# nikhilTkur/Multigrid_dolfinx

Measured on AMD Instinct MI355X. Metric: V-cycles/sec + achieved HBM GB/s, 3D Poisson P1 1024³ DoF, 1/2/4/8 MI355X, higher is better.
Workload: dtype f64

## Files before the change

multigrid_dolfinx_amd/csrc/mg_capi.hip:

```cpp
#include "../../include/mg_hip.h"
#include "mg_csr_check.h"
#include "mg_kernels.hip.h"
#include "mg_direct.hip.h"
#include "mg_jacobi2.hip.h"
#include "mg_jacobik3d.hip.h"
#include "mg_jacobiblk.hip.h"
#include "mg_lattice.hip.h"
#include "mg_diffusion_mf.hip.h"
#include "mg_diffusion_adj.hip.h"
#include "mg_diffusion_kappa.hip.h"

#include <dlfcn.h>
#include <rccl/rccl.h>

#include <algorithm>
#include <array>
#include <cmath>
#include <cstdio>
#include <cstdlib>
#include <cstring>
#include <string>
#include <type_traits>
#include <vector>

// ... 216 lines not shown
    double *pcg_r = nullptr, *pcg_z = nullptr, *pcg_q = nullptr, *pcg_part_a = nullptr, *pcg_part_b = nullptr;
    DVector pcg_p;
    int pcg_parts = 0, pcg_parts_a = 0;
    int pcg_predict = 0;
    double* fcg_work = nullptr;
    double* fcg_spmv = nullptr;
    int64_t fcg_work_n = 0, fcg_spmv_n = 0;
    int use_graph = 1;
    int comm_priority = 1;
    int lattice_march = 1;
    int64_t lattice_march_min_rows = 1 << 22;
    int lattice_gs2 = 0;
    int diffusion_faces = MG_FACES_ALL;
    int dkappa_gather = 0;
    int lattice_tile = 0;
    int lattice_segments = 0;
    int slab_pair_form = 0;
    int graph_comm = 0;
    uint64_t epoch = 1;
    std::vector<CycleGraph> graphs;
    bool capturing = false;
    int use_direct = 1;
    int require_diagonal = 1;
    int fuse_restrict = 1;
    int fuse_block = 1;
    int64_t fuse_block_min_rows = (int64_t)1 << 15, fuse_block_max_rows = (int64_t)1 << 23;
    int fuse_block_k = 0, fuse_block_ez = 11;
    int direct_block_rows = 2048;
    int fuse_2d_lines = 0;
    int gen_odd_rows = 0;
    int cls_escape = 1;
    int storage_auto = 1;
    int storage_qbits = 0;
    int use_classes = 1;
    int fuse_sweeps = 1;
    int64_t fuse_min_rows = (int64_t)1 << 24;
    int fuse_segments = 0;
    int fuse_nontemporal = 0;
    int fuse_classes = 1;
    int fuse_plain_shape = 0;
    int fuse_plain = 2;
    int class_sweeps = 1;
    int fuse_k = 5;
    int fuse_k_shape = -1;
    int fuse_k_segments = 0;
    int timing_force_form = -1;
    int64_t fuse_k_slab_min_rows = (int64_t)1 << 20;
    int fuse_k_slab_min_sweeps = 4;
    int64_t fuse_k_min_rows = (int64_t)1 << 24;
    int64_t fuse_k_small_rows = (int64_t)1 << 22;
    int64_t fuse_k5_min_rows = (int64_t)1 << 26;
    int64_t fuse_k4_min_rows = 0;
    int fuse_k_nt_store = 0;
    int fuse_k_tail = 1;
    int fuse_k_small_tiles = 0;
    int fuse_k_pf = 1;
    int fuse_k_dpp = 1;
    std::vector<const void*> large_lds_kernels;
    int fuse_shape = 1;
    int fuse_wi = 0;
    int fuse_even = 0;
    int march_sweeps = 1;
    int64_t march_min_rows = (int64_t)1 << 22;
    int march_shape = 0;
    int64_t fuse_small_2d_rows = 2048;
    int fuse_small = 1;
    int fuse_2d = 1;
    int fuse_2d_k = 5;
    int fuse_xcd_chunk = 32;
    int cls_blocks_per_cu = 4;
    DirectSolver direct;
    int* ptab_count = nullptr;
    int p1_prolong = 0;
    int* rtab_count = nullptr;
    int* rtab_off = nullptr;
    double* rtab_w = nullptr;
    int rtab_m = 0;
    int* ptab_off = nullptr;
    double* ptab_w = nullptr;
    Level mass;
    int mass_level = -1;
    DVector mass_out, diff, uexact;
    int uexact_level = -1;
    int64_t uploads = 0, downloads = 0, graph_replays = 0;
    struct SmootherCount { int64_t launches = 0, sweeps = 0, tail = 0; };
    std::vector<std::array<SmootherCount, MG_PATH_COUNT>> smoother_counts;
    int jk3_tail = 0;
    double* stage = nullptr;
    int64_t stage_elems = 0;
    int64_t bytes = 0;
    Comm comm;
    hipDeviceProp_t prop{};
};

namespace {

constexpr int kMaxParts = 1024;

template <class T>
int dev_alloc(mg_context* c, T** p, size_t count) {
    *p = nullptr;
    if (count == 0) count = 1;
    HIP_TRY(hipMalloc(reinterpret_cast<void**>(p), count * sizeof(T)));
    c->bytes += (int64_t)(count * sizeof(T));
    return 0;
}
// ... 692 lines not shown
    HIP_TRY(hipStreamSynchronize(c->stream));
    if (cm.ar(cm.user, cm.h_stage, count) != 0) return fail("allreduce callback failed");
    HIP_TRY(hipMemcpyAsync(dev, cm.h_stage, (size_t)count * 8, hipMemcpyHostToDevice, c->stream));
    HIP_TRY(hipStreamSynchronize(c->stream));
    return 0;
}

int allgather_planes(mg_context* c, const std::vector<int>& splits, int64_t plane, double* full) {
    Comm& cm = c->comm;
    if (!cm.active()) return 0;
    if (cm.nccl) {
        NCCL_TRY(g_rccl.GroupStart());
        for (int r = 0; r < cm.world; ++r) {
            double* seg = full + (int64_t)splits[r] * plane;
            const size_t cnt = (size_t)(splits[r + 1] - splits[r]) * (size_t)plane;
            NCCL_TRY(g_rccl.Broadcast(seg, seg, cnt, ncclDouble, r, cm.nccl, c->stream));
        }
        NCCL_TRY(g_rccl.GroupEnd());
        return 0;
    }
    if (!cm.ag) return fail("no transport configured");
    const int64_t total = (int64_t)splits[cm.world] * plane;
    const int64_t mine = (int64_t)(splits[cm.rank + 1] - splits[cm.rank]) * plane;
    MG_TRY(ensure_host_stage(c, (size_t)(total + mine)));
    double* h_send = cm.h_stage + total;
    HIP_TRY(hipMemcpyAsync(h_send, full + (int64_t)splits[cm.rank] * plane, (size_t)mine * 8, hipMemcpyDeviceToHost,
                           c->stream));
    HIP_TRY(hipStreamSynchronize(c->stream));
    std::vector<int64_t> counts(cm.world);
    for (int r = 0; r < cm.world; ++r) counts[r] = (int64_t)(splits[r + 1] - splits[r]) * plane;
    if (cm.ag(cm.user, h_send, mine, cm.h_stage, counts.data()) != 0) return fail("allgatherv callback failed");
    HIP_TRY(hipMemcpyAsync(full, cm.h_stage, (size_t)total * 8, hipMemcpyHostToDevice, c->stream));
    HIP_TRY(hipStreamSynchronize(c->stream));
    return 0;
}

DVector* pick(Level& L, int which) {
    switch (which) {
        case MG_VEC_V: return &L.v;
        case MG_VEC_F: return &L.f;
        case MG_VEC_R: return &L.v2;
        case MG_VEC_ERR: return &L.err;
        default: return nullptr;
    }
}

int64_t min_slab_rows(const Level& L) {
    if (L.replicated || L.splits.size() < 2) return L.nloc;
    int nk = INT32_MAX;
    for (size_t r = 0; r + 1 < L.splits.size(); ++r) nk = std::min(nk, L.splits[r + 1] - L.splits[r]);
    return (int64_t)nk * L.g.plane;
}

bool fused_sweeps_ok(const mg_context* c, const Level& L, bool ignore_size = false) {
    if (!c->fuse_sweeps || !L.sdia || L.wu != 4 || L.flat) return false;
    if (L.g.nx < 32 || L.g.ny < 32 || min_slab_rows(L) < 8 * L.g.plane) return false;
    if (L.up[1] != 1 || L.up[2] != L.g.nx || (int64_t)L.up[3] != L.g.plane) return false;
    return ignore_size || min_slab_rows(L) >= c->fuse_min_rows;
}

int launch_lat_gs2(mg_context* c, const Level& L, int c1, int c2, const double* xold_rows, double* xnew_rows) {
    Gs2Args a{};
    a.xold = xold_rows; a.xnew = xnew_rows; a.f = L.f.rows;
    a.cls = L.scls; a.s_pack = L.s_pack; a.s_val = L.s_val; a.s_cnt = L.s_cnt;
    a.W = L.W; a.WP = (L.W + 3) / 4 * 4 + 4; a.ntop = L.lm_ntop;
    for (int t = 0; t < LM_K; ++t) a.top[t] = L.lm_top[t];
    a.nloc = L.nloc; a.P = L.g.plane; a.nx = L.g.nx; a.ny = L.g.ny; a.nz = L.g.nk;
    a.c1 = c1; a.c2 = c2; a.omega = c->omega;
    a.ntx = (L.g.nx + G2_TI - 1) / G2_TI; a.nty = (L.g.ny + G2_TJ - 1) / G2_TJ;
    const int64_t ntile = (int64_t)a.ntx * a.nty;
    const int64_t resident = 2 * (int64_t)std::max(1, c->prop.multiProcessorCount);
    int nseg = c->lattice_segments;
    if (nseg <= 0 && 2 * ntile >= resident) nseg = (int)std::max<int64_t>(1, (13 * resident / 2 + ntile - 1) / ntile);
    if (nseg <= 0) nseg = best_segments(ntile, resident, L.g.nk, L.g.nk / 16, 12.0);
    nseg = std::max(1, std::min(nseg, std::max(1, L.g.nk / 16)));
    a.seglen = (L.g.nk + nseg - 1) / nseg;
    nseg = (L.g.nk + a.seglen - 1) / a.seglen;
    const int64_t items = ntile * nseg;
    a.xcd_chunk = 16;
    unsigned grid = 0;
    MG_TRY(tile_grid(items, a.xcd_chunk, &grid));
    a.nitems = (unsigned)items;
    const size_t lds = g2_lds_bytes(L.W);
    if (lds > (size_t)80 * 1024) return fail("lattice march: class tables too wide");
    MG_TRY(allow_large_lds(c, reinterpret_cast<const void*>(lat_gs2), (size_t)80 * 1024));
    hipLaunchKernelGGL(lat_gs2, dim3(grid), dim3(G2_THREADS), lds, c->stream, a);
    HIP_TRY(hipGetLastError());
    return 0;
}

int allow_large_lds(mg_context* c, const void* kernel, size_t bytes) {
    if (std::find(c->large_lds_kernels.begin(), c->large_lds_kernels.end(), kernel) != c->large_lds_kernels.end()) return 0;
    HIP_TRY(hipFuncSetAttribute(kernel, hipFuncAttributeMaxDynamicSharedMemorySize, (int)bytes));
    c->large_lds_kernels.push_back(kernel);
    return 0;
}

constexpr int kJ2Lines = 16;

struct J2Plan { int ntx, nty, nseg, zb, seglen, wi; };

int jacobi2_lines(const mg_context* c, const Level& L) {
    const int sh = c->fuse_shape;
    if (!(cls_full(L) && c->fuse_classes)) return (c->fuse_plain == 2 && c->fuse_plain_shape == 0) ? 12 : kJ2Lines;
    return (sh == 1 || sh == 3) ? 24 : kJ2Lines;
}

J2Plan jacobi2_plan(const mg_context* c, const Level& L, bool slab, int64_t boundary_rows) {
    J2Plan p{};
// ... 167 lines not shown
    HIP_TRY(hipStreamSynchronize(c->stream));
    std::vector<int> map(512, 0);
    int ncls = L.ncls;
    bool grown = false;
    for (int side = 0; side < 2 && ok; ++side) {
        if (!(side == 0 ? lo : hi)) continue;
        const double* t = theirs.data() + (size_t)side * nt;
        const int n_theirs = (int)t[0];
        if (n_theirs <= 0 || n_theirs > 256) { ok = 0; break; }
        for (int j = 0; j < n_theirs && ok; ++j) {
            const double* row = t + 8 + (size_t)j * CLS_W;
            int found = -1;
            for (int i = 0; i < ncls && found < 0; ++i)
                if (std::memcmp(mine.data() + 8 + (size_t)i * CLS_W, row, 7 * sizeof(double)) == 0) found = i;
            if (found < 0) {
                if (ncls >= 256) { ok = 0; break; }
                std::memcpy(mine.data() + 8 + (size_t)ncls * CLS_W, row, 7 * sizeof(double));
                mine[8 + (size_t)ncls * CLS_W + 7] = 0.0;
                found = ncls++;
                grown = true;
            }
            map[(size_t)side * 256 + j] = found;
        }
    }
    double flag = ok ? 0.0 : 1.0;
    HIP_TRY(hipMemcpyAsync(c->scalars + 7, &flag, sizeof(double), hipMemcpyHostToDevice, c->stream));
    MG_TRY(allreduce_sum(c, c->scalars + 7, 1));
    HIP_TRY(hipMemcpyAsync(&flag, c->scalars + 7, sizeof(double), hipMemcpyDeviceToHost, c->stream));
    HIP_TRY(hipStreamSynchronize(c->stream));
    if (flag != 0.0) return 0;
    if (grown) {
        HIP_TRY(hipMemcpyAsync(L.ctab, mine.data() + 8, 256 * CLS_W * sizeof(double), hipMemcpyHostToDevice, c->stream));
        L.ncls = ncls;
    }
    HIP_TRY(hipMemcpyAsync(dmap.p, map.data(), 512 * sizeof(int), hipMemcpyHostToDevice, c->stream));
    const int* dm = reinterpret_cast<const int*>(dmap.p);
    if (lo) hipLaunchKernelGGL(doubles_to_classes, dim3(nb), dim3(256), 0, c->stream, recv.p, dm, L.cls + L.cls_lead - (int64_t)n, (int64_t)n);
    if (hi) hipLaunchKernelGGL(doubles_to_classes, dim3(nb), dim3(256), 0, c->stream, recv.p + n, dm + 256, L.cls + L.cls_lead + L.nloc, (int64_t)n);
    HIP_TRY(hipGetLastError());
    HIP_TRY(hipStreamSynchronize(c->stream));
    L.cls_halo = 1;
    return 0;
}

bool sweepsk_ok(const mg_context* c, const Level& L, bool ignore_size = false) {
    if (c->fuse_k < 3 || !L.cls || !c->fuse_classes) return false;
    if (L.cls_escape) {
        if (L.esc_kmax < 3) return false;
        ignore_size = true;
    }
    const bool slab = is_slab(c, L);
    if (slab && (L.hd < 2 || L.cls_halo < 0 || c->halo_planes != 1)) return false;
    if (!ignore_size && (slab ? min_slab_rows(L) < c->fuse_k_slab_min_rows : L.nloc < c->fuse_k_min_rows)) return false;
    return fused_sweeps_ok(c, L, true) && L.g.nk >= 8;
}

int sweepsk_max(const mg_context* c, const Level& L) {
    const int k = std::min(std::min(c->fuse_k, 5), L.nloc < c->fuse_k4_min_rows ? 3 : L.nloc < c->fuse_k_small_rows ? 5 : L.nloc < c->fuse_k5_min_rows ? 4 : 5);
    return L.cls_escape ? std::min(k, L.esc_kmax) : k;
}

template <int K>
int escape_window_k(mg_context* c, const Level& L, const unsigned char* cls, int64_t clead, unsigned* most) {
    constexpr int WI = 64 - 2 * K, HY = 16 * 2 - 2 * K + 2;
    JK3WindowArgs a{};
    a.cls = cls; a.clead = clead; a.P = L.g.plane; a.nx = L.g.nx; a.ny = L.g.ny; a.nz = L.g.nk;
    a.ntx = (a.nx + WI - 1) / WI; a.nty = (a.ny + HY - 1) / HY;
    a.most = reinterpret_cast<unsigned*>(c->partials);
    HIP_TRY(hipMemsetAsync(a.most, 0, sizeof(unsigned), c->stream));
    hipLaunchKernelGGL((jk3_escape_window<K, 16, 2, 1>), dim3((unsigned)(a.ntx * a.nty)), dim3(256), 0, c->stream, a);
    HIP_TRY(hipGetLastError());
    HIP_TRY(hipMemcpyAsync(most, a.most, sizeof(unsigned), hipMemcpyDeviceToHost, c->stream));
    HIP_TRY(hipStreamSynchronize(c->stream));
    if (std::getenv("MG_DEBUG_STORAGE"))
        std::fprintf(stderr, "[mg] escape rows: at most %u in %d planes of a tile (%d sweeps per pass, pool of %d)\n", *most, K + 2, K, jk3_pool(K));
    return 0;
}

int escape_kmax(mg_context* c, const Level& L, const unsigned char* cls, int64_t clead, int* kmax) {
    *kmax = 0;
    if (L.wu != 4 || L.g.nk < 8 || L.g.nx < 32 || L.g.ny < 32) return 0;
    unsigned most = 0;
    MG_TRY(escape_window_k<5>(c, L, cls, clead, &most));
    if (most <= (unsigned)jk3_pool(5)) { *kmax = 5; return 0; }
    MG_TRY(escape_window_k<4>(c, L, cls, clead, &most));
    if (most <= (unsigned)jk3_pool(4)) { *kmax = 4; return 0; }
    MG_TRY(escape_window_k<3>(c, L, cls, clead, &most));
    if (most <= (unsigned)jk3_pool(3)) *kmax = 3;
    return 0;
}

struct JK3Range { int za0, za1, zb0, zb1; };

int jk3_shape(const mg_context* c, int K) {
    return c->fuse_k_shape >= 0 ? c->fuse_k_shape : (K >= 5 ? 8 : 7);
}

template <int K, int NW, int LPW, int M, bool DPP, int PF = 1, int WPE = (NW == 12 ? 3 : 2), int TR = 256, bool ESC = false, bool B1 = false>
int launch_jacobikc_t(mg_context* c, JK3Args a, bool finest, const JK3Range& zr, int seglen) {
    constexpr int EX = 64 * M, EY = NW * LPW, WI = EX - 2 * K, HY = EY - 2 * K + 2;
    a.ntx = (a.nx + WI - 1) / WI;
    a.nty = (a.ny + HY - 1) / HY;
    const int64_t ntile = (int64_t)a.ntx * a.nty;
    constexpr size_t lds = B1 ? jk3b_lds_bytes<K, NW, LPW, M, TR>() : jk3_lds_bytes<K, NW, LPW, M, TR, ESC>();
    static_assert(lds <= 160 * 1024, "one CU's LDS");
    a.za0 = zr.za0; a.za1 = zr.za1; a.zb0 = zr.zb0; a.zb1 = zr.zb1;
    const int planes = std::max(0, zr.za1 - zr.za0) + std::max(0, zr.zb1 - zr.zb0);
// ... 2329 lines not shown
    } else if (k == "lattice_march") {
        c->lattice_march = value != 0;
    } else if (k == "lattice_march_min_rows") {
        c->lattice_march_min_rows = value;
    } else if (k == "dkappa_gather") {
        c->dkappa_gather = value != 0;
    } else if (k == "lattice_gs2") {
        c->lattice_gs2 = value != 0;
    } else if (k == "lattice_tile") {
        if (value < 0 || value > 2) return fail("lattice_tile must be 0, 1 or 2");
        c->lattice_tile = (int)value;
    } else if (k == "lattice_segments") {
        if (value < 0 || value > 4096) return fail("lattice_segments must be in 0..4096");
        c->lattice_segments = (int)value;
    } else if (k == "fuse_xcd_chunk") {
        if (value < 1 || value > 512) return fail("fuse_xcd_chunk must be in 1..512");
        c->fuse_xcd_chunk = (int)value;
    } else if (k == "cls_blocks_per_cu") {
        if (value < 1 || value > 64) return fail("cls_blocks_per_cu must be in 1..64");
        c->cls_blocks_per_cu = (int)value;
    } else if (k == "fuse_wi") {
        c->fuse_wi = (int)value;
    } else if (k == "fuse_even") {
        c->fuse_even = value != 0;
    } else if (k == "class_sweeps") {
        c->class_sweeps = value != 0;
    } else if (k == "fuse_plain_shape") {
        if (value < 0 || value > 2) return fail("fuse_plain_shape must be 0..2");
        c->fuse_plain_shape = (int)value;
    } else if (k == "fuse_plain") {
        if (value != 1 && value != 2) return fail("fuse_plain must be 1 or 2");
        c->fuse_plain = (int)value;
    } else if (k == "fuse_k") {
        if (value < 0 || value > 5) return fail("fuse_k must be in 0..5 (below 3: pairs of sweeps only)");
        c->fuse_k = (int)value;
    } else if (k == "fuse_k_shape") {
        if (value < -1 || value > 8) return fail("fuse_k_shape must be 0..8, or -1 (by sweeps per pass)");
        c->fuse_k_shape = (int)value;
    } else if (k == "fuse_k_slab_min_rows") {
        c->fuse_k_slab_min_rows = value;
    } else if (k == "fuse_k_slab_min_sweeps") {
        if (value < 2) return fail("fuse_k_slab_min_sweeps must be at least 2");
        c->fuse_k_slab_min_sweeps = (int)value;
    } else if (k == "fuse_k_min_rows") {
        c->fuse_k_min_rows = value;
    } else if (k == "fuse_k_small_rows") {
        c->fuse_k_small_rows = value;
    } else if (k == "fuse_k5_min_rows") {
        c->fuse_k5_min_rows = value;
    } else if (k == "fuse_k4_min_rows") {
        c->fuse_k4_min_rows = value;
    } else if (k == "fuse_k_nt_store") {
        c->fuse_k_nt_store = value != 0;
    } else if (k == "fuse_k_tail") {
        if (value < 0) return fail("fuse_k_tail must be >= 0");
        c->fuse_k_tail = (int)value;
    } else if (k == "fuse_k_small_tiles") {
        c->fuse_k_small_tiles = value != 0;
    } else if (k == "fuse_k_pf") {
        if (value != 1 && value != 2) return fail("fuse_k_pf must be 1 or 2");
        c->fuse_k_pf = (int)value;
    } else if (k == "fuse_k_dpp") {
        c->fuse_k_dpp = value != 0;
    } else if (k == "fuse_k_segments") {
        if (value < 0) return fail("fuse_k_segments must be >= 0");
        c->fuse_k_segments = (int)value;
    } else if (k == "fuse_classes") {
        c->fuse_classes = value != 0;
    } else if (k == "fuse_nontemporal") {
        c->fuse_nontemporal = value != 0;
    } else if (k == "fuse_segments") {
        if (value < 0) return fail("fuse_segments must be >= 0");
        c->fuse_segments = (int)value;
    } else if (k == "coarse_direct") {
        c->use_direct = value != 0;
        free_direct(c);
    } else if (k == "pcg_chunk") {
        if (value < 1) return fail("pcg_chunk must be positive");
        c->pcg_chunk = (int)value;
    } else {
        return fail("unknown tuning key " + k);
    }
    return 0;
}

namespace {

int upload_permutation(mg_context* c, Level& L, const int64_t* grid_index, int64_t n_rows) {
    if (!grid_index) return 0;
    std::vector<int> p32((size_t)n_rows);
    std::vector<char> seen((size_t)n_rows, 0);
    for (int64_t d = 0; d < n_rows; ++d) {
        const int64_t p = grid_index[d];
        if (p < 0 || p >= n_rows || seen[(size_t)p]) return fail("grid_index is not a permutation of the grid nodes");
        seen[(size_t)p] = 1;
        p32[(size_t)d] = (int)p;
    }
    MG_TRY(dev_alloc(c, &L.perm, (size_t)n_rows));
    HIP_TRY(hipMemcpy(L.perm, p32.data(), (size_t)n_rows * 4, hipMemcpyHostToDevice));
    return 0;
}

int build_level_from_csr(mg_context* c, int level, Level& L, int64_t n_rows, int64_t nnz, const void* indptr,
                         int indptr_is_64, const int32_t* indices, const double* data, const int64_t* grid_index,
                         int prune_zeros, bool vectors = true, const int64_t* local_cols = nullptr, int64_t n_cols = 0,
                         bool device_csr = false) {
// ... 1303 lines not shown
```

multigrid_dolfinx_amd/csrc/mg_jacobik3d.hip.h:

```cpp
#pragma once
#include "mg_jacobi2.hip.h"
#include <type_traits>

namespace mgk {

struct JK3Args {
    const double* x;
    const double* f;
    double* out;
    const unsigned char* cls;
    const double* ctab;
    int64_t clead, P;
    int ncls, cmain;
    double cm[8];
    double omega;
    int nx, ny, nz;
    int plo, phi;
    int ntx, nty, seglen, za0, za1, zb0, zb1;
    int ta, seglen_b;
    unsigned nitems, xcd_chunk;
    int nt_store;
    int escape;
    const double* dvals;
    int64_t mlead;
    int sshift;
    int force_form;
};

constexpr int jk3_pool(int K) { return K >= 5 ? 512 : 1024; }

template <int K, int NW, int LPW, int M, int TR> constexpr size_t jk3_lds_doubles() {
    return TR * CLS_W + (size_t)K * (NW * LPW + 2) * (64 * M) + 2 * (64 * M + 2);
}
template <int K, int NW, int LPW, int M, int TR> constexpr size_t jk3b_lds_doubles() {
    return TR * CLS_W + (size_t)(2 * (K - 1) * (NW * LPW + 1) + 1) * (64 * M);
}
template <int K, int NW, int LPW, int M, int TR> constexpr size_t jk3b_lds_bytes() {
    return sizeof(double) * jk3b_lds_doubles<K, NW, LPW, M, TR>();
}

template <int K, int NW, int LPW, int M, int TR, bool ESC = false> constexpr size_t jk3_lds_bytes() {
    constexpr size_t base = jk3_lds_doubles<K, NW, LPW, M, TR>();
    return sizeof(double) * (ESC ? (base + CLS_W - 1) / CLS_W * CLS_W + (size_t)(jk3_pool(K) + 1) * CLS_W : base);
}


template <int K, int NW, int LPW, int M, bool DPP, int PF, int TR, bool ESC = false, bool B1 = false>
__device__ __forceinline__ void jk3_body(const JK3Args& a) {
    constexpr int EX = 64 * M, EY = NW * LPW, NC = M * LPW, IMG = (EY + 2) * EX;
    constexpr int IS = (EY + 1) * EX, PS = (K - 1) * IS;
    static_assert(!B1 || (DPP && PF == 1 && !ESC), "one barrier per step: DPP neighbours, one plane of x in flight, no escape rows");
    constexpr int CBITS = ESC ? 16 : 8, CPR = 32 / CBITS, CW = (NC + CPR - 1) / CPR;
    constexpr unsigned CMASK = (1u << CBITS) - 1u;
    constexpr int DYN0 = (int)((jk3_lds_doubles<K, NW, LPW, M, TR>() + CLS_W - 1) / CLS_W);
    static_assert(CLS_W == 8, "table rows of eight doubles");
    constexpr int WI = EX - 2 * K, HY = EY - 2 * K + 2;
    static_assert(NC * (K + 1) <= 64, "the fast-path flags live in one scalar register pair");
    static_assert(WI > 0 && HY > 0, "tile too small for K sweeps");
    static_assert(PF == 1 || PF == 2, "planes of x in flight");
    extern __shared__ double j2_smem[];
    double* const sT = j2_smem;
    double* const sI = sT + TR * CLS_W + (EX + 2);
    const int lane = threadIdx.x & 63;
    const int wave = __builtin_amdgcn_readfirstlane((int)(threadIdx.x >> 6));

    unsigned id;
    {
        const unsigned b = blockIdx.x, xcd = b & 7u, j = b >> 3, ch = a.xcd_chunk;
        id = ((j / ch) * 8u + xcd) * ch + (j % ch);
    }
    if (id >= a.nitems) return;
    const unsigned ntile = (unsigned)(a.ntx * a.nty);
    const int nsa = (a.za1 - a.za0 + a.seglen - 1) / a.seglen;
    const int nsb = (a.zb1 - a.zb0 + a.seglen - 1) / a.seglen;
    const unsigned items_a = (unsigned)a.ta * (unsigned)(nsa + max(nsb, 0));
    unsigned tt;
    int z0, z1;
    if (id < items_a) {
        const int seg = (int)(id / (unsigned)a.ta);
        tt = id % (unsigned)a.ta;
        z0 = seg < nsa ? a.za0 + seg * a.seglen : a.zb0 + (seg - nsa) * a.seglen;
        z1 = min(seg < nsa ? a.za1 : a.zb1, z0 + a.seglen);
    } else {
        const unsigned j = id - items_a, tb = ntile - (unsigned)a.ta;
        tt = (unsigned)a.ta + j % tb;
        z0 = a.za0 + (int)(j / tb) * a.seglen_b;
        z1 = min(a.za1, z0 + a.seglen_b);
    }
    const int tiy = (int)(tt / (unsigned)a.ntx), tix = (int)(tt % (unsigned)a.ntx);
    if (z1 <= z0) return;
    const int tx0 = tix * WI - K, ty0 = tiy * HY - (K - 1);

    {
        const int nt = a.ncls * CLS_W;
        for (int i = threadIdx.x; i < nt; i += NW * WAVE) {
            double v = a.ctab[i];
            if ((i & (CLS_W - 1)) == CLS_W - 1) {
                const double d = a.ctab[i - 4];
                v = a.omega * (1.0 / (d != 0.0 ? d : 1.0));
            }
            sT[i] = v;
        }
        constexpr int NZ = B1 ? (2 * (K - 1) * (EY + 1) + 1) * EX : K * IMG + 2 * (EX + 2);
        for (int i = threadIdx.x; i < NZ; i += NW * WAVE) sT[TR * CLS_W + i] = 0.0;
    }
    unsigned* const esc_count = reinterpret_cast<unsigned*>(sT + (size_t)CLS_W * (DYN0 + jk3_pool(K)));
    if constexpr (ESC) {
        if (threadIdx.x == 0) *esc_count = 0u;
    }
    const double m0 = a.cm[0], m1 = a.cm[1], m2 = a.cm[2], m3 = a.cm[3], m4 = a.cm[4], m5 = a.cm[5], m6 = a.cm[6];
    const double mcf = a.omega * (1.0 / (m3 != 0.0 ? m3 : 1.0));
    const int cmain = a.cmain;

    const int ey0 = wave * LPW;
    const int lw0 = (ey0 + 1) * EX + lane;
    auto lwof = [&](int c) -> int { return (c / M) * EX + 64 * (c % M); };
    int ibase[(K + 1) / 2];
#pragma unroll
    for (int q = 0; q < (K + 1) / 2; ++q) {
        ibase[q] = 2 * q * IMG + lw0;
        asm volatile("" : "+v"(ibase[q]));
    }
    auto image = [&](int t) -> double* { return sI + ibase[t >> 1] + (t & 1) * IMG; };
    int bcur = 0, bprev = 0;
    auto limg = [&](int base, int t) -> double* { return j2_smem + base + (t - 1) * IS + EX; };
    double XP[B1 ? NC : 1];
    double hS[M], hN[M];
    unsigned inT = 0;
    const int64_t rb0 = (int64_t)(ty0 + ey0) * a.nx + (tx0 + lane);
    auto rowof = [&](int c) -> int64_t { return rb0 + (int64_t)(c / M) * a.nx + 64 * (c % M); };
    unsigned shw = 0;
#pragma unroll
    for (int c = 0; c < NC; ++c) {
        const int ex = lane + 64 * (c % M), ey = ey0 + c / M;
        if (ex >= K && ex < EX - K && ey >= K - 1 && ey <= EY - K && tx0 + ex < a.nx && ty0 + ey < a.ny) inT |= 1u << c;
        const int64_t r = rowof(c);
        shw |= (r < 0 ? 0u : (r >= a.P ? 2u : 1u)) << (2 * c);
    }
    auto shof = [&](int c) -> int { return (int)((shw >> (2 * c)) & 3u) - 1; };
    unsigned standin = 0;
#pragma unroll
    for (int c = 0; c < NC; ++c) {
        const int line = ty0 + ey0 + c / M;
        if (lane + 64 * (c % M) > a.nx + 1 - tx0 || line < -2 || line > a.ny + 1) standin |= 1u << c;
    }
    const bool wlo = wave == 0, whi = wave == NW - 1;

    const int bias = 2 * a.nx + K + 2;
    const int xcl = a.nx + 1 - tx0;
    unsigned eo[NC], eor[M];
#pragma unroll
    for (int c = 0; c < NC; ++c)
        eo[c] = 8u * (unsigned)(min(max(ty0 + ey0 + c / M, -2), a.ny + 1) * a.nx + tx0 + min(lane + 64 * (c % M), xcl) + bias);
#pragma unroll
    for (int r = 0; r < M; ++r)
        eor[r] = 8u * (unsigned)((wlo ? max(ty0 - 1, -2) : min(ty0 + EY, a.ny + 1)) * a.nx + tx0 + min(lane + 64 * r, xcl) + bias);
    unsigned eos[B1 ? M : 1], eon[B1 ? M : 1];
    if constexpr (B1) {
#pragma unroll
        for (int r = 0; r < M; ++r) {
            eos[r] = 8u * (unsigned)(min(max(ty0 + ey0 - 1, -2), a.ny + 1) * a.nx + tx0 + min(lane + 64 * r, xcl) + bias);
            eon[r] = 8u * (unsigned)(min(max(ty0 + ey0 + LPW, -2), a.ny + 1) * a.nx + tx0 + min(lane + 64 * r, xcl) + bias);
        }
    }
    const unsigned char* const clsb = a.cls + a.clead - bias;
    const double* const xb0 = a.x - bias;
    const double* const fb0 = a.f - bias;
    auto sbase = [](const void* p) -> gcptr_t {
        const unsigned long long u = (unsigned long long)p;
        const unsigned lo = (unsigned)__builtin_amdgcn_readfirstlane((int)(unsigned)u);
        const unsigned hi = (unsigned)__builtin_amdgcn_readfirstlane((int)(unsigned)(u >> 32));
        return (gcptr_t)(((unsigned long long)hi << 32) | lo);
    };
    auto ldd = [](gcptr_t b, unsigned e8) -> double {
        asm volatile("" : "+v"(e8));
        return *(const __attribute__((address_space(1))) double*)(b + e8);
    };
    typedef unsigned int __attribute__((aligned(1))) u32_unaligned_t;
    auto ldc = [](gcptr_t b, unsigned e8) -> int {
        unsigned e = e8 >> 3;
        asm volatile("" : "+v"(e));
        return (int)*(const __attribute__((address_space(1))) u32_unaligned_t*)(b + e);
    };
    const int pmin = -a.plo - 1, pmax = a.nz + a.phi;

    double acc[K][NC], fr[K][NC];
    double XA[NC], XB[PF == 2 ? NC : 1], hyA[M], hyB[PF == 2 ? M : 1];
    int CA[NC], CB[PF == 2 ? NC : 1];
    double FN[PF == 2 ? NC : 1];
    unsigned cw[K + 1][CW];
    unsigned long long fast = 0;
    constexpr unsigned long long ALLFAST = (NC * (K + 1) == 64) ? ~0ull : ((1ull << (NC * (K + 1))) - 1ull);
#pragma unroll
    for (int c = 0; c < NC; ++c) {
#pragma unroll
        for (int t = 0; t < K; ++t) acc[t][c] = fr[t][c] = 0.0;
        XA[c] = 0.0;
        CA[c] = 0;
    }
// ... 3 lines not shown
        for (int q = 0; q < CW; ++q) cw[j][q] = 0u;
#pragma unroll
    for (int r = 0; r < M; ++r) hyA[r] = hS[r] = hN[r] = 0.0;
    XB[0] = 0.0; hyB[0] = 0.0; CB[0] = 0; FN[0] = 0.0;
#pragma unroll
    for (int c = 0; c < (B1 ? NC : 1); ++c) XP[c] = 0.0;

    auto load_slice = [&](const int i, const int n, const int plane, const int fplane, double (&X)[NC], int (&C)[NC], double (&hy)[M])
        __attribute__((always_inline)) {
        const int64_t o = (int64_t)min(max(plane, pmin), pmax) * a.P;
        const gcptr_t cb = sbase(clsb + o);
        const gcptr_t xb = sbase(xb0 + o);
        const gcptr_t fb = sbase(fb0 + (int64_t)min(max(fplane, pmin), pmax) * a.P);
#pragma unroll
        for (int c = 0; c < NC; ++c) {
            if ((c * n) / NC != i) continue;
            X[c] = ldd(xb, eo[c]);
            C[c] = ldc(cb, eo[c]);
            if constexpr (PF == 2) FN[c] = ldd(fb, eo[c]);
            else fr[K - 1][c] = ldd(fb, eo[c]);
        }
        if constexpr (B1) {
            if (i == n - 1) {
#pragma unroll
                for (int r = 0; r < M; ++r) { hS[r] = ldd(xb, eos[r]); hN[r] = ldd(xb, eon[r]); }
            }
        } else if (i == n - 1 && (wlo || whi)) {
#pragma unroll
            for (int r = 0; r < M; ++r) hy[r] = ldd(xb, eor[r]);
        }
    };
    auto cls_of = [&](int j, int c) -> int { return (int)((cw[j][c / CPR] >> (CBITS * (c % CPR))) & CMASK); };
    auto cls_now = [&](int j, int c) -> int {
        unsigned w = cw[j][c / CPR];
        asm volatile("" : "+v"(w));
        return (int)((w >> (CBITS * (c % CPR))) & CMASK);
    };
    int k_plane = 0;
    bool k_store = false;
    __attribute__((address_space(1))) char* k_out = nullptr;
    auto store = [&](int c, double v) {
        unsigned e8 = eo[c];
        asm volatile("" : "+v"(e8));
        if (a.nt_store) __builtin_nontemporal_store(v, (__attribute__((address_space(1))) double*)(k_out + e8));
        else *(__attribute__((address_space(1))) double*)(k_out + e8) = v;
    };
    int lo_t[K + 1], n_t[K + 1];
#pragma unroll
    for (int t = 1; t <= K; ++t) {
        lo_t[t] = -min(a.plo, K - t);
        n_t[t] = a.nz + min(a.phi, K - t) - lo_t[t];
    }

    auto phase_a_fast = [&](auto col_tag, const double (&X)[NC]) __attribute__((always_inline)) {
        constexpr bool COL = decltype(col_tag)::value;
#pragma unroll
        for (int r = 0; r < M; ++r) {
#pragma unroll
            for (int l = 0; l < LPW; ++l) {
                const int c = l * M + r, iw = lwof(c);
                double k0 = m0, k6 = m6, kcf = mcf;
                if constexpr (COL) {
                    const dvec2_t* const tr = reinterpret_cast<const dvec2_t*>(sT + CLS_W * cls_of(0, c));
                    const dvec2_t t01 = tr[0], t67 = tr[3];
                    k0 = t01.x; k6 = t67.x; kcf = t67.y;
                }
                double nw = X[c];
#pragma unroll
                for (int t = 1; t <= K; ++t) {
                    if constexpr (B1) {
                        const double wd = t == 1 ? XP[c] : limg(bprev, t - 1)[iw];
                        const double s = fma(k6, nw, acc[t - 1][c]);
                        const double o = wd + kcf * (fr[K - t][c] - s);
                        acc[t - 1][c] = fma(k0, wd, 0.0);
                        if (t > 1) limg(bcur, t - 1)[iw] = nw;
                        nw = o;
                        continue;
                    }
                    double* const img = image(t - 1);
                    const double wd = img[iw];
                    const double s = fma(k6, nw, acc[t - 1][c]);
                    const double o = wd + kcf * (fr[K - t][c] - s);
                    acc[t - 1][c] = fma(k0, wd, 0.0);
                    img[iw] = nw;
                    nw = o;
                }
                if (k_store && (inT >> c & 1u)) store(c, nw);
            }
        }
    };
    auto phase_b_fast = [&](auto col_tag, const int t, const double (&X)[NC]) __attribute__((always_inline)) {
        constexpr bool COL = decltype(col_tag)::value;
        const double* const img = B1 ? limg(bcur, t > 1 ? t - 1 : 1) : image(t - 1);
        double v[LPW][M], ys[M], yn[M];
#pragma unroll
        for (int r = 0; r < M; ++r) {
            if (B1 && t == 1) {
                ys[r] = hS[r];
#pragma unroll
                for (int l = 0; l < LPW; ++l) v[l][r] = X[l * M + r];
                yn[r] = hN[r];
                continue;
            }
            ys[r] = img[-EX + 64 * r];
#pragma unroll
            for (int l = 0; l < LPW; ++l) v[l][r] = img[l * EX + 64 * r];
            yn[r] = img[LPW * EX + 64 * r];
        }
#pragma unroll
        for (int l = 0; l < LPW; ++l) {
            double yw[M], ye[M];
            if constexpr (DPP) {
                double fw[M], fe[M];
#pragma unroll
                for (int r = 0; r < M; ++r) { fw[r] = jk3_from_west(v[l][r]); fe[r] = jk3_from_east(v[l][r]); }
#pragma unroll
                for (int r = 0; r < M; ++r) {
                    yw[r] = (r > 0 && lane == 0) ? fw[r > 0 ? r - 1 : 0] : fw[r];
                    ye[r] = (r + 1 < M && lane == 63) ? fe[r + 1 < M ? r + 1 : r] : fe[r];
                }
            } else {
#pragma unroll
                for (int r = 0; r < M; ++r) {
                    yw[r] = img[l * EX + 64 * r - 1];
                    ye[r] = img[l * EX + 64 * r + 1];
                }
            }
#pragma unroll
            for (int r = 0; r < M; ++r) {
                const int c = l * M + r;
                double k1 = m1, k2 = m2, k3 = m3, k4 = m4, k5 = m5;
                if constexpr (COL) {
                    const dvec2_t* const tr = reinterpret_cast<const dvec2_t*>(sT + CLS_W * cls_of(0, c));
                    const dvec2_t t01 = tr[0], t23 = tr[1], t45 = tr[2];
                    k1 = t01.y; k2 = t23.x; k3 = t23.y; k4 = t45.x; k5 = t45.y;
                }
                double s = acc[t - 1][c];
                s = fma(k1, l > 0 ? v[l > 0 ? l - 1 : 0][r] : ys[r], s);
                s = fma(k2, yw[r], s);
                s = fma(k3, v[l][r], s);
                s = fma(k4, ye[r], s);
                s = fma(k5, l + 1 < LPW ? v[l + 1 < LPW ? l + 1 : l][r] : yn[r], s);
                acc[t - 1][c] = s;
            }
        }
    };
    auto phase_a_general = [&](const double (&X)[NC]) __attribute__((always_inline)) {
#pragma unroll
        for (int c = 0; c < NC; ++c) {
            const int iw = lwof(c);
            double nw = X[c];
            int pc = k_plane + shof(c);
            asm volatile("" : "+v"(pc));
#pragma unroll
            for (int t = 1; t <= K; ++t) {
                const int j = K - t;
                double* const img = B1 ? limg(bcur, t > 1 ? t - 1 : 1) : image(t - 1);
                const double wd = B1 ? (t == 1 ? XP[B1 ? c : 0] : limg(bprev, t - 1)[iw]) : img[iw];
                const dvec2_t t67 = reinterpret_cast<const dvec2_t*>(sT + CLS_W * cls_now(j, c))[3];
                const dvec2_t t01 = reinterpret_cast<const dvec2_t*>(sT + CLS_W * cls_now(j + 1, c))[0];
                const double s = fma(t67.x, nw, acc[t - 1][c]);
                double o = wd + t67.y * (fr[j][c] - s);
                o = (unsigned)(pc + j - lo_t[t]) < (unsigned)n_t[t] ? o : 0.0;
                acc[t - 1][c] = fma(t01.x, wd, 0.0);
                if (!B1 || t > 1) img[iw] = nw;
                nw = o;
                __builtin_amdgcn_sched_barrier(0);
            }
            if (k_store && (inT >> c & 1u)) store(c, nw);
        }
    };
    auto phase_b_general = [&](const int t, const double (&X)[NC]) __attribute__((always_inline)) {
        double x0w[B1 ? NC : 1], x0e[B1 ? NC : 1];
        if constexpr (B1) {
            if (t == 1) {
                double fw[NC], fe[NC];
#pragma unroll
                for (int c = 0; c < NC; ++c) { fw[c] = jk3_from_west(X[c]); fe[c] = jk3_from_east(X[c]); }
#pragma unroll
                for (int c = 0; c < NC; ++c) {
                    const int r = c % M;
                    x0w[c] = (r > 0 && lane == 0) ? fw[r > 0 ? c - 1 : c] : fw[c];
                    x0e[c] = (r + 1 < M && lane == 63) ? fe[r + 1 < M ? c + 1 : c] : fe[c];
                }
            }
        }
#pragma unroll
        for (int c = 0; c < NC; ++c) {
            const int iw = lwof(c);
            double ys, yw, yd, ye, yn;
            if (B1 && t == 1) {
                const int l = c / M, r = c % M;
                ys = l > 0 ? X[l > 0 ? c - M : c] : hS[r];
                yw = x0w[B1 ? c : 0]; yd = X[c]; ye = x0e[B1 ? c : 0];
                yn = l + 1 < LPW ? X[l + 1 < LPW ? c + M : c] : hN[r];
            } else {
                const double* const img = B1 ? limg(bcur, t > 1 ? t - 1 : 1) : image(t - 1);
                ys = img[iw - EX]; yw = img[iw - 1]; yd = img[iw]; ye = img[iw + 1]; yn = img[iw + EX];
            }
            const dvec2_t* const tr = reinterpret_cast<const dvec2_t*>(sT + CLS_W * cls_now(K - t, c));
            const dvec2_t t01 = tr[0], t23 = tr[1], t45 = tr[2];
            double s = acc[t - 1][c];
            s = fma(t01.y, ys, s);
            s = fma(t23.x, yw, s);
            s = fma(t23.y, yd, s);
            s = fma(t45.x, ye, s);
            s = fma(t45.y, yn, s);
            acc[t - 1][c] = s;
            __builtin_amdgcn_sched_barrier(0);
        }
    };

    auto step = [&](const int k, double (&X)[NC], int (&C)[NC], double (&hy)[M], double (&XN)[PF == 2 ? NC : 1],
                    int (&CN)[PF == 2 ? NC : 1], double (&hyN)[PF == 2 ? M : 1]) __attribute__((always_inline)) {
        k_plane = k; k_store = k >= z0;
        if constexpr (B1) {
            bcur = TR * CLS_W + ey0 * EX + lane + (k & 1) * PS;
            bprev = TR * CLS_W + ey0 * EX + lane + ((k + 1) & 1) * PS;
            asm volatile("" : "+v"(bcur));
            asm volatile("" : "+v"(bprev));
        }
        {
            const unsigned long long u = (unsigned long long)(a.out - bias + (int64_t)k * a.P);
            const unsigned lo = (unsigned)__builtin_amdgcn_readfirstlane((int)(unsigned)u);
            const unsigned hi = (unsigned)__builtin_amdgcn_readfirstlane((int)(unsigned)(u >> 32));
            k_out = (__attribute__((address_space(1))) char*)(((unsigned long long)hi << 32) | lo);
        }
#pragma unroll
        for (int c = 0; c < NC; ++c) {
            asm volatile("" : "+v"(C[c]));
            asm volatile("" : "+v"(X[c]));
            C[c] &= 255;
        }
        if constexpr (ESC) {
            if (a.escape) {
                const int64_t mp = (int64_t)min(max(k + K, pmin), pmax) * a.P - bias + a.mlead;
                const int sh = a.sshift;
                const double* const dv = a.dvals;
                auto at = [&](int64_t m, int slot) -> double { return dv[((((m >> sh) << 2) + slot) << sh) + (m & (((int64_t)1 << sh) - 1))]; };
                unsigned long long em[NC];
                unsigned total = 0u;
// ... 7 lines not shown
                    unsigned b0 = 0u;
                    if (lane == 0) b0 = atomicAdd(esc_count, total);
                    b0 = (unsigned)__builtin_amdgcn_readfirstlane((int)b0);
                    double e[NC][7];
#pragma unroll
                    for (int c = 0; c < NC; ++c) {
                        if (C[c] == CLS_ESCAPE) {
                            const int64_t m = mp + (int64_t)(eo[c] >> 3);
                            e[c][0] = at(m - a.P, 3); e[c][1] = at(m - a.nx, 2); e[c][2] = at(m - 1, 1);
                            e[c][3] = at(m, 0); e[c][4] = at(m, 1); e[c][5] = at(m, 2); e[c][6] = at(m, 3);
                        }
                    }
#pragma unroll
                    for (int c = 0; c < NC; ++c) {
                        if (C[c] == CLS_ESCAPE) {
                            const unsigned below = __builtin_amdgcn_mbcnt_hi((unsigned)(em[c] >> 32), __builtin_amdgcn_mbcnt_lo((unsigned)em[c], 0u));
                            const int row = DYN0 + (int)((b0 + below) & (unsigned)(jk3_pool(K) - 1));
                            double* const tr = sT + CLS_W * row;
#pragma unroll
                            for (int i = 0; i < 7; ++i) tr[i] = e[c][i];
                            tr[7] = a.omega * (1.0 / (e[c][3] != 0.0 ? e[c][3] : 1.0));
                            C[c] = row;
                        }
                        b0 += (unsigned)__popcll(em[c]);
                    }
                }
            }
        }
        {
            unsigned m = 0;
#pragma unroll
            for (int q = 0; q < CW; ++q) cw[K][q] = 0u;
#pragma unroll
            for (int c = 0; c < NC; ++c) {
                cw[K][c / CPR] |= (unsigned)C[c] << (CBITS * (c % CPR));
                if (__builtin_amdgcn_readfirstlane((int)(__ballot(C[c] != cmain) == 0ull))) m |= 1u << c;
            }
            fast |= (unsigned long long)m << (K * NC);
        }
        int form = 2;
        if ((a.plo > 0 || k >= 1) && (a.phi > 0 || k + K + 1 < a.nz)) {
            if (fast == ALLFAST) {
                form = 0;
            } else {
                bool same = true;
#pragma unroll
                for (int j = 0; j <= K; ++j)
#pragma unroll
                    for (int c = 0; c < NC; ++c) same = same && cls_of(j, c) == cls_of(0, c);
                if (__builtin_amdgcn_readfirstlane((int)(__ballot(!same) == 0ull))) form = 1;
            }
        }
        if (a.force_form >= 0) form = a.force_form;
        if (form == 0) phase_a_fast(std::false_type{}, X);
        else if (form == 1) phase_a_fast(std::true_type{}, X);
        else phase_a_general(X);
        if constexpr (B1) {
#pragma unroll
            for (int c = 0; c < NC; ++c) XP[c] = X[c];
        } else if (wlo || whi) {
            double* const ring = image(0) + (wlo ? -EX : LPW * EX);
#pragma unroll
            for (int r = 0; r < M; ++r) ring[64 * r] = hy[r];
        }
#pragma unroll
        for (int c = 0; c < NC; ++c) {
#pragma unroll
            for (int j = 0; j + 1 < K; ++j) fr[j][c] = fr[j + 1][c];
            asm volatile("" : "+v"(fr[K - 2][c]));
        }
#pragma unroll
        for (int j = 0; j < K; ++j)
#pragma unroll
            for (int q = 0; q < CW; ++q) cw[j][q] = cw[j + 1][q];
        fast >>= NC;
        __syncthreads();
        if constexpr (PF == 2) {
#pragma unroll
            for (int c = 0; c < NC; ++c) {
                X[c] = XN[c]; C[c] = CN[c]; fr[K - 1][c] = FN[c];
                asm volatile("" : "+v"(X[c]));
                asm volatile("" : "+v"(C[c]));
                asm volatile("" : "+v"(fr[K - 1][c]));
            }
            if (wlo || whi) {
#pragma unroll
                for (int r = 0; r < M; ++r) { hy[r] = hyN[r]; asm volatile("" : "+v"(hy[r])); }
            }
        }
        auto issue = [&](const int i, const int n) __attribute__((always_inline)) {
            __builtin_amdgcn_sched_barrier(0);
            if constexpr (PF == 2) load_slice(i, n, k + K + 2, k + K + 1, XN, CN, hyN);
            else load_slice(i, n, k + K + 1, k + K, X, C, hy);
            __builtin_amdgcn_sched_barrier(0);
        };
#pragma unroll
        for (int t = 1; t <= K; ++t) {
            if (form == 0) phase_b_fast(std::false_type{}, t, X);
            else if (form == 1) phase_b_fast(std::true_type{}, t, X);
            else phase_b_general(t, X);
            issue(t - 1, K);
        }
        if constexpr (!B1) __syncthreads();
    };

    load_slice(0, 1, z0 - K, z0 - K - 1, XA, CA, hyA);
    if constexpr (PF == 2) {
#pragma unroll
        for (int c = 0; c < NC; ++c) fr[K - 1][c] = FN[c];
        load_slice(0, 1, z0 - K + 1, z0 - K, XB, CB, hyB);
    }
    __syncthreads();

    for (int k = z0 - 2 * K; k < z1; ++k) step(k, XA, CA, hyA, XB, CB, hyB);
}

template <int K, int NW, int LPW, int M, bool DPP, int PF, int WPE, int TR>
__global__ __attribute__((amdgpu_flat_work_group_size(NW * WAVE, NW * WAVE), amdgpu_waves_per_eu(WPE, WPE)))
void sdia_jacobikc(JK3Args a) {
    jk3_body<K, NW, LPW, M, DPP, PF, TR>(a);
}

template <int K, int NW, int LPW, int M, bool DPP, int PF, int WPE, int TR>
__global__ __attribute__((amdgpu_flat_work_group_size(NW * WAVE, NW * WAVE), amdgpu_waves_per_eu(WPE, WPE)))
void sdia_jacobikc_finest(JK3Args a) {
    jk3_body<K, NW, LPW, M, DPP, PF, TR>(a);
}

template <int K, int NW, int LPW, int M, int WPE, int TR>
__global__ __attribute__((amdgpu_flat_work_group_size(NW * WAVE, NW * WAVE), amdgpu_waves_per_eu(WPE, WPE)))
void sdia_jacobikc_b1(JK3Args a) {
    jk3_body<K, NW, LPW, M, true, 1, TR, false, true>(a);
}
template <int K, int NW, int LPW, int M, int WPE, int TR>
__global__ __attribute__((amdgpu_flat_work_group_size(NW * WAVE, NW * WAVE), amdgpu_waves_per_eu(WPE, WPE)))
void sdia_jacobikc_finest_b1(JK3Args a) {
    jk3_body<K, NW, LPW, M, true, 1, TR, false, true>(a);
}

template <int K, int NW, int LPW, int M, bool DPP, int PF, int WPE, int TR>
__global__ __attribute__((amdgpu_flat_work_group_size(NW * WAVE, NW * WAVE), amdgpu_waves_per_eu(WPE, WPE)))
void sdia_jacobikc_escape(JK3Args a) {
    jk3_body<K, NW, LPW, M, DPP, PF, TR, true>(a);
}

struct JK3WindowArgs {
    const unsigned char* cls;
    int64_t clead, P;
    int nx, ny, nz, ntx, nty;
    unsigned* most;
};

template <int K, int NW, int LPW, int M>
// ... 29 lines not shown
```

Before: 4.319.

## Skip dead halo-row sweeps in temporally blocked Jacobi kernel and add side-size knob

Adds compile-time per-row sweep caps for the single-block (B1, 16-wave, 2 lines per wave) temporal-blocking Jacobi kernel. Rows near the y-edges of a tile only need to be updated up to their distance from the edge, so the fast and general phases now skip sweeps past that cap and write the last valid value into the image. Edge waves are specialised through a dispatch lambda to keep the caps constexpr. A new fuse_k_min_side option (default 32, so the old behaviour) can let the fused K-sweep path run on smaller grids. The specialisation adds code size and branch divergence between waves, and it can raise register pressure.

```diff
diff --git a/multigrid_dolfinx_amd/csrc/mg_capi.hip b/multigrid_dolfinx_amd/csrc/mg_capi.hip
--- a/multigrid_dolfinx_amd/csrc/mg_capi.hip
+++ b/multigrid_dolfinx_amd/csrc/mg_capi.hip
@@ -292,6 +292,7 @@
     int64_t fuse_k5_min_rows = (int64_t)1 << 26;
     int64_t fuse_k4_min_rows = 0;
     int fuse_k_nt_store = 0;
+    int fuse_k_min_side = 32;
     int fuse_k_tail = 1;
     int fuse_k_small_tiles = 0;
     int fuse_k_pf = 1;
@@ -1090,9 +1091,9 @@
     return (int64_t)nk * L.g.plane;
 }
 
-bool fused_sweeps_ok(const mg_context* c, const Level& L, bool ignore_size = false) {
+bool fused_sweeps_ok(const mg_context* c, const Level& L, bool ignore_size = false, int min_side = 32) {
     if (!c->fuse_sweeps || !L.sdia || L.wu != 4 || L.flat) return false;
-    if (L.g.nx < 32 || L.g.ny < 32 || min_slab_rows(L) < 8 * L.g.plane) return false;
+    if (L.g.nx < min_side || L.g.ny < min_side || min_slab_rows(L) < 8 * L.g.plane) return false;
     if (L.up[1] != 1 || L.up[2] != L.g.nx || (int64_t)L.up[3] != L.g.plane) return false;
     return ignore_size || min_slab_rows(L) >= c->fuse_min_rows;
 }
@@ -1366,7 +1367,8 @@
     const bool slab = is_slab(c, L);
     if (slab && (L.hd < 2 || L.cls_halo < 0 || c->halo_planes != 1)) return false;
     if (!ignore_size && (slab ? min_slab_rows(L) < c->fuse_k_slab_min_rows : L.nloc < c->fuse_k_min_rows)) return false;
-    return fused_sweeps_ok(c, L, true) && L.g.nk >= 8;
+    const int side = slab || L.cls_escape ? 32 : c->fuse_k_min_side;
+    return fused_sweeps_ok(c, L, true, side) && L.g.nk >= 8;
 }
 
 int sweepsk_max(const mg_context* c, const Level& L) {
@@ -3802,6 +3804,9 @@
         c->fuse_k4_min_rows = value;
     } else if (k == "fuse_k_nt_store") {
         c->fuse_k_nt_store = value != 0;
+    } else if (k == "fuse_k_min_side") {
+        if (value < 16 || value > 32) return fail("fuse_k_min_side must be in 16..32");
+        c->fuse_k_min_side = (int)value;
     } else if (k == "fuse_k_tail") {
         if (value < 0) return fail("fuse_k_tail must be >= 0");
         c->fuse_k_tail = (int)value;
diff --git a/multigrid_dolfinx_amd/csrc/mg_jacobik3d.hip.h b/multigrid_dolfinx_amd/csrc/mg_jacobik3d.hip.h
--- a/multigrid_dolfinx_amd/csrc/mg_jacobik3d.hip.h
+++ b/multigrid_dolfinx_amd/csrc/mg_jacobik3d.hip.h
@@ -45,6 +45,14 @@
 }
 
 
+template <int K, int EY, int E0> struct jk3_caps {
+    static constexpr int of(int l) {
+        if (E0 < 0) return K;
+        const int ey = E0 + l, a = ey + 1 < EY - ey ? ey + 1 : EY - ey;
+        return a < K ? a : K;
+    }
+};
+
 template <int K, int NW, int LPW, int M, bool DPP, int PF, int TR, bool ESC = false, bool B1 = false>
 __device__ __forceinline__ void jk3_body(const JK3Args& a) {
     constexpr int EX = 64 * M, EY = NW * LPW, NC = M * LPW, IMG = (EY + 2) * EX;
@@ -145,6 +153,36 @@
         if (lane + 64 * (c % M) > a.nx + 1 - tx0 || line < -2 || line > a.ny + 1) standin |= 1u << c;
     }
     const bool wlo = wave == 0, whi = wave == NW - 1;
+    constexpr bool CAPS = B1 && NW == 16 && LPW == 2 && M == 1 && K >= 3;
+    using caps_all = jk3_caps<K, EY, -1>;
+    using caps_w0 = jk3_caps<K, EY, 0>;
+    using caps_w1 = jk3_caps<K, EY, LPW>;
+    using caps_w2 = jk3_caps<K, EY, EY - 2 * LPW>;
+    using caps_w3 = jk3_caps<K, EY, EY - LPW>;
+    constexpr bool CAPS1 = CAPS && (caps_w1::of(0) < K || caps_w1::of(LPW - 1) < K);
+    constexpr bool CAPS2 = CAPS && (caps_w2::of(0) < K || caps_w2::of(LPW - 1) < K);
+    const int wkind = !CAPS ? 0 : wave == 0 ? 1 : wave == NW - 1 ? 4 : (CAPS1 && wave == 1) ? 2 : (CAPS2 && wave == NW - 2) ? 3 : 0;
+    auto by_caps = [&](auto&& fn) __attribute__((always_inline)) {
+        if constexpr (CAPS) {
+            if (__builtin_expect(wkind != 0, 0)) {
+                if (wkind == 1) fn(caps_w0{});
+                else if (wkind == 4) fn(caps_w3{});
+                else if constexpr (CAPS1 && CAPS2) {
+                    if (wkind == 2) fn(caps_w1{});
+                    else fn(caps_w2{});
+                }
+                return;
+            }
+        }
+        fn(caps_all{});
+    };
+    auto cap_of = [&](int c) -> int {
+        if constexpr (!CAPS) return K;
+        const int ey = ey0 + c / M;
+        int cap = min(min(ey + 1, EY - ey), K);
+        asm volatile("" : "+v"(cap));
+        return __builtin_amdgcn_readfirstlane(cap);
+    };
 
     const int bias = 2 * a.nx + K + 2;
     const int xcl = a.nx + 1 - tx0;
@@ -254,8 +292,9 @@
         n_t[t] = a.nz + min(a.phi, K - t) - lo_t[t];
     }
 
-    auto phase_a_fast = [&](auto col_tag, const double (&X)[NC]) __attribute__((always_inline)) {
+    auto phase_a_fast = [&](auto col_tag, auto caps, const double (&X)[NC]) __attribute__((always_inline)) {
         constexpr bool COL = decltype(col_tag)::value;
+        using CAP = decltype(caps);
 #pragma unroll
         for (int r = 0; r < M; ++r) {
 #pragma unroll
@@ -270,6 +309,10 @@
                 double nw = X[c];
 #pragma unroll
                 for (int t = 1; t <= K; ++t) {
+                    if (t > CAP::of(l)) {
+                        if (t == CAP::of(l) + 1) (B1 ? limg(bcur, t - 1) : image(t - 1))[iw] = nw;
+                        continue;
+                    }
                     if constexpr (B1) {
                         const double wd = t == 1 ? XP[c] : limg(bprev, t - 1)[iw];
                         const double s = fma(k6, nw, acc[t - 1][c]);
@@ -287,12 +330,13 @@
                     img[iw] = nw;
                     nw = o;
                 }
-                if (k_store && (inT >> c & 1u)) store(c, nw);
-            }
-        }
-    };
-    auto phase_b_fast = [&](auto col_tag, const int t, const double (&X)[NC]) __attribute__((always_inline)) {
+                if (CAP::of(l) == K && k_store && (inT >> c & 1u)) store(c, nw);
+            }
+        }
+    };
+    auto phase_b_fast = [&](auto col_tag, auto caps, const int t, const double (&X)[NC]) __attribute__((always_inline)) {
         constexpr bool COL = decltype(col_tag)::value;
+        using CAP = decltype(caps);
         const double* const img = B1 ? limg(bcur, t > 1 ? t - 1 : 1) : image(t - 1);
         double v[LPW][M], ys[M], yn[M];
 #pragma unroll
@@ -311,6 +355,7 @@
         }
 #pragma unroll
         for (int l = 0; l < LPW; ++l) {
+            if (t > CAP::of(l)) continue;
             double yw[M], ye[M];
             if constexpr (DPP) {
                 double fw[M], fe[M];
@@ -354,10 +399,15 @@
             double nw = X[c];
             int pc = k_plane + shof(c);
             asm volatile("" : "+v"(pc));
+            const int cap = cap_of(c);
 #pragma unroll
             for (int t = 1; t <= K; ++t) {
                 const int j = K - t;
                 double* const img = B1 ? limg(bcur, t > 1 ? t - 1 : 1) : image(t - 1);
+                if (CAPS && t > cap) {
+                    if (t == cap + 1) img[iw] = nw;
+                    continue;
+                }
                 const double wd = B1 ? (t == 1 ? XP[B1 ? c : 0] : limg(bprev, t - 1)[iw]) : img[iw];
                 const dvec2_t t67 = reinterpret_cast<const dvec2_t*>(sT + CLS_W * cls_now(j, c))[3];
                 const dvec2_t t01 = reinterpret_cast<const dvec2_t*>(sT + CLS_W * cls_now(j + 1, c))[0];
@@ -389,6 +439,7 @@
         }
 #pragma unroll
         for (int c = 0; c < NC; ++c) {
+            if (CAPS && t > cap_of(c)) continue;
             const int iw = lwof(c);
             double ys, yw, yd, ye, yn;
             if (B1 && t == 1) {
@@ -502,9 +553,15 @@
             }
         }
         if (a.force_form >= 0) form = a.force_form;
-        if (form == 0) phase_a_fast(std::false_type{}, X);
-        else if (form == 1) phase_a_fast(std::true_type{}, X);
-        else phase_a_general(X);
+        if constexpr (CAPS) {
+            if (form == 0) by_caps([&](auto caps) __attribute__((always_inline)) { phase_a_fast(std::false_type{}, caps, X); });
+            else if (form == 1) by_caps([&](auto caps) __attribute__((always_inline)) { phase_a_fast(std::true_type{}, caps, X); });
+            else phase_a_general(X);
+        } else {
+            if (form == 0) phase_a_fast(std::false_type{}, caps_all{}, X);
+            else if (form == 1) phase_a_fast(std::true_type{}, caps_all{}, X);
+            else phase_a_general(X);
+        }
         if constexpr (B1) {
 #pragma unroll
             for (int c = 0; c < NC; ++c) XP[c] = X[c];
@@ -546,9 +603,15 @@
         };
 #pragma unroll
         for (int t = 1; t <= K; ++t) {
-            if (form == 0) phase_b_fast(std::false_type{}, t, X);
-            else if (form == 1) phase_b_fast(std::true_type{}, t, X);
-            else phase_b_general(t, X);
+            if constexpr (CAPS) {
+                if (form == 0) by_caps([&](auto caps) __attribute__((always_inline)) { phase_b_fast(std::false_type{}, caps, t, X); });
+                else if (form == 1) by_caps([&](auto caps) __attribute__((always_inline)) { phase_b_fast(std::true_type{}, caps, t, X); });
+                else phase_b_general(t, X);
+            } else {
+                if (form == 0) phase_b_fast(std::false_type{}, caps_all{}, t, X);
+                else if (form == 1) phase_b_fast(std::true_type{}, caps_all{}, t, X);
+                else phase_b_general(t, X);
+            }
             issue(t - 1, K);
         }
         if constexpr (!B1) __syncthreads();
```

New measurement: 4.436 (median of 6 runs). +2.7%, better.
